# CentaureaHO/CTC-VR

Hardware: AMD Instinct MI355X
Metric: audio-frames/sec, streaming RNN-T greedy decode (higher is better)
Workload: dtype bf16x3; 1 GPU; configs[1]: batch=64/GPU synthetic 10 s 80-dim fbank, streaming chunk=16 (online_rnnt_decode.py semantics), greedy decode, whole-utterance call (tokens identical to the per-chunk API); streams_per_gpu=64, chunk_frames=16, chunks=62, weights=seeded synthetic (seed 0, blank_bias 12.0), parallelism=streams sharded x1, no data-path collective

## Files before the change

### ctc-vr_amd/csrc/api_lifecycle.hip.inc

```

int rnnt_abi_version(void) { return 3; }

const char* rnnt_last_error(const rnnt_ctx* ctx) { return ctx ? ctx->err.c_str() : "null context"; }

int rnnt_create(const rnnt_config* cfg, rnnt_ctx** out) {
    if (!cfg || !out) return RNNT_ERR_ARG;
    *out = nullptr;
    rnnt_ctx* ctx = new rnnt_ctx();
    ctx->cfg = *cfg;
    *out = ctx;
    if (cfg->max_streams < 1 || cfg->max_chunk_frames < 7 || cfg->max_cache_frames < 1 || cfg->max_cache_frames > RNNT_PE_LEN ||
        cfg->max_enc_frames < 1 || cfg->max_tokens < 1 || cfg->vocab_size < 2 || cfg->blank_id < 0 || cfg->blank_id >= cfg->vocab_size ||
        cfg->n_steps < 1 || cfg->max_beam < 0 || cfg->max_beam > 64)
        return fail(ctx, RNNT_ERR_ARG, "rnnt_create: bad config");
    HIPCHK(hipSetDevice(cfg->device));
    if (const char* ng = getenv("RNNT_NO_GRAPH")) ctx->use_graphs = (ng[0] == '1') ? 0 : 1;
    if (const char* pe = getenv("RNNT_PERSISTENT")) ctx->use_persistent = (pe[0] == '0') ? 0 : 1;
    if (const char* me = getenv("RNNT_DEC_MULTI")) ctx->use_multi = (me[0] == '0') ? 0 : 1;
    HIPCHK(hipDeviceGetAttribute(&ctx->n_cus, hipDeviceAttributeMultiprocessorCount, cfg->device));
    if (const char* ae = getenv("RNNT_ATTN_STREAM")) ctx->attn_stream = (ae[0] == '0') ? 0 : 1;
    if (const char* be = getenv("RNNT_BEAM_CHAIN")) ctx->use_beam_chain = (be[0] == '0') ? 0 : 1;
    if (const char* pg = getenv("RNNT_PREFIX_GROUP")) ctx->prefix_group = pg[0] == '1' ? 1 : (pg[0] == '4' ? 4 : 0);
    if (const char* fu = getenv("RNNT_FUSED")) ctx->use_fused = atoi(fu);
    if (const char* fe = getenv("RNNT_FUSE_AFTER_NORM")) ctx->fuse_after_norm = (fe[0] == '0') ? 0 : 1;
// ... 325 lines not shown
        putv(&ctx->whh_il, hh);
        putv(&ctx->wih_il, ih);
        putv(&ctx->b_lstm_il, bb);
        put(&ctx->pred_embed, emb->data.data(), emb->data.size());
        put(&ctx->wpr, wpr->data.data(), wpr->data.size()); put(&ctx->bpr, bpr->data.data(), D);
        put(&ctx->wenc, wen->data.data(), wen->data.size()); put(&ctx->benc, ben->data.data(), D);
        put(&ctx->wpf, wpf->data.data(), wpf->data.size()); put(&ctx->bpf, bpf->data.data(), D);
        put(&ctx->wout, wou->data.data(), wou->data.size()); put(&ctx->bout, bou->data.data(), V);
        std::vector<float> wc((size_t)D * D), bc(D);
        for (int n = 0; n < D; ++n) {
            for (int k = 0; k < D; ++k) {
                double acc = 0.0;
                for (int j = 0; j < D; ++j) acc += (double)wpf->data[(size_t)n * D + j] * (double)wpr->data[(size_t)j * D + k];
                wc[(size_t)n * D + k] = (float)acc;
            }
            double acc = bpf->data[n];
            for (int j = 0; j < D; ++j) acc += (double)wpf->data[(size_t)n * D + j] * (double)bpr->data[j];
            bc[n] = (float)acc;
        }
        putv(&ctx->wjc, wc);
        putv(&ctx->bjc, bc);
        const HostTensor* cw = find(ctx, "ctc_head.ctc_lo.weight");
        const HostTensor* cb = find(ctx, "ctc_head.ctc_lo.bias");
        ctx->wctc = ctx->bctc = nullptr;
        if (cw && cb && cw->dims == std::vector<int64_t>{V, D} && cb->dims == std::vector<int64_t>{V}) {
            put(&ctx->wctc, cw->data.data(), cw->data.size());
            put(&ctx->bctc, cb->data.data(), V);
        }
    }
#undef NEED
    while (blob.size() % 8) blob.push_back(0.f);
    int rc;
    if (ctx->blob.cap != blob.size()) {
        HIPCHK(hipStreamSynchronize(s));
        ctx->blob_hi.release();
        ctx->blob_lo.release();
        if ((rc = reserve_exact(ctx, ctx->blob, blob.size()))) return rc;
    }
    HIPCHK(hipMemcpyAsync(ctx->blob, blob.data(), blob.size() * sizeof(float), hipMemcpyHostToDevice, s));
    for (auto& f : fix) *f.first = ctx->blob + f.second;
    ctx->numerics = RNNT_NUM_F32;
    if (numerics_mode != RNNT_NUMERICS_FP32) {
        if ((rc = reserve(ctx, ctx->blob_hi, blob.size()))) return rc;
        if ((rc = reserve(ctx, ctx->blob_lo, blob.size()))) return rc;
        const long long n8 = (long long)(blob.size() / 8);
        if (numerics_mode == RNNT_NUMERICS_F16X3) hipLaunchKernelGGL(split_planes<true>, dim3(grid_for(n8)), dim3(256), 0, s, ctx->blob, ctx->blob_hi, ctx->blob_lo, n8);
        else hipLaunchKernelGGL(split_planes<false>, dim3(grid_for(n8)), dim3(256), 0, s, ctx->blob, ctx->blob_hi, ctx->blob_lo, n8);
        LAUNCHCHK("split_planes");
    }
    {
        const int nm = numerics_mode;
        const size_t per_w = nm == RNNT_NUMERICS_BF16 ? 8 : 4;
        const size_t layer_w = (size_t)4 * FF * D + 5 * D * D + 2 * D * D;
        const size_t vecs = ((size_t)L * layer_w + (size_t)D * 2304) / per_w;
        if (ctx->fuse_w.cap != vecs) {
            HIPCHK(hipStreamSynchronize(s));
            if ((rc = reserve_exact(ctx, ctx->fuse_w, vecs))) return rc;
        }
        if ((rc = reserve(ctx, ctx->layers_dev, (size_t)L))) return rc;
        std::vector<LayerDev> ld(L);
        uint4* cur = ctx->fuse_w;
        auto pack = [&](const float* W, int N, int K) -> const uint4* {
            const uint4* out = cur;
            const long long total = (long long)((N + 15) / 16) * (K / 32) * 64;
            const dim3 g(grid_for(total)), b(256);
            switch (nm) {
                case RNNT_NUMERICS_BF16X3: hipLaunchKernelGGL(pack_frag<RNNT_NUM_BF16X3>, g, b, 0, s, W, N, K, K, cur); break;
                case RNNT_NUMERICS_BF16: hipLaunchKernelGGL(pack_frag<RNNT_NUM_BF16>, g, b, 0, s, W, N, K, K, cur); break;
                case RNNT_NUMERICS_F16X3: hipLaunchKernelGGL(pack_frag<RNNT_NUM_F16X3>, g, b, 0, s, W, N, K, K, cur); break;
                default: hipLaunchKernelGGL(pack_frag<RNNT_NUM_F32>, g, b, 0, s, W, N, K, K, cur); break;
            }
            cur += (size_t)N * K / per_w;
            return out;
        };
        for (int l = 0; l < L; ++l) {
            const LayerW& w = ctx->lw[l];
            LayerDev& d = ld[l];
            d.w1m = pack(w.w1m, FF, D); d.w2m = pack(w.w2m, D, FF); d.wq = pack(w.wq, D, D); d.wk = pack(w.wk, D, D); d.wv = pack(w.wv, D, D);
            d.wo = pack(w.wo, D, D); d.pw1 = pack(w.pw1, 2 * D, D); d.pw2 = pack(w.pw2, D, D); d.w1 = pack(w.w1, FF, D); d.w2 = pack(w.w2, D, FF);
            d.b1m = w.b1m; d.b2m = w.b2m; d.bq = w.bq; d.bk = w.bk; d.bv = w.bv; d.bo = w.bo; d.bpw1 = w.bpw1; d.bpw2 = w.bpw2; d.b1 = w.b1; d.b2 = w.b2;
            d.ln_ffm_g = w.ln_ffm_g; d.ln_ffm_b = w.ln_ffm_b; d.ln_mha_g = w.ln_mha_g; d.ln_mha_b = w.ln_mha_b; d.ln_conv_g = w.ln_conv_g;
            d.ln_conv_b = w.ln_conv_b; d.ln_ff_g = w.ln_ff_g; d.ln_ff_b = w.ln_ff_b; d.ln_fin_g = w.ln_fin_g; d.ln_fin_b = w.ln_fin_b;
            d.wdw_t = w.wdw_t; d.bdw = w.bdw; d.bn_s = w.bn_s; d.bn_t = w.bn_t;
            d.kc = ctx->kcache + (size_t)l * ctx->cfg.max_streams * ctx->tcap * D;
            d.vc = ctx->vcache + (size_t)l * ctx->cfg.max_streams * ctx->tcap * D;
            d.gr = ctx->gring + (size_t)l * ctx->cfg.max_streams * ctx->cap * D;
            d.xr = ctx->xring + (size_t)l * ctx->cfg.max_streams * ctx->cap * D;
        }
        ctx->conv2_wp = pack(ctx->conv2_w, D, 2304);
        LAUNCHCHK("pack_frag");
        HIPCHK(hipMemcpyAsync(ctx->layers_dev, ld.data(), L * sizeof(LayerDev), hipMemcpyHostToDevice, s));
        ctx->layers_host = ld;
        HIPCHK(hipStreamSynchronize(s));
    }
    if (numerics_mode != RNNT_NUMERICS_FP32 && V <= JR_NT * 16 && V % 4 == 0) {
        const bool lo = numerics_mode != RNNT_NUMERICS_BF16;
        const size_t bytes = (size_t)(lo ? 16 : 8) * JR_SLOT;
        if (ctx->joint_wfrag.cap != bytes) {
            HIPCHK(hipStreamSynchronize(s));
            if ((rc = reserve_exact(ctx, ctx->joint_wfrag, bytes))) return rc;
        }
        if ((rc = reserve(ctx, ctx->joint_counter, (size_t)4))) return rc;
        const dim3 g((unsigned)(bytes / 16 + 255) / 256), b(256);
        if (numerics_mode == RNNT_NUMERICS_F16X3) hipLaunchKernelGGL((pack_joint_w<true, true>), g, b, 0, s, ctx->wout, (int)V, ctx->joint_wfrag);
        else if (lo) hipLaunchKernelGGL((pack_joint_w<false, true>), g, b, 0, s, ctx->wout, (int)V, ctx->joint_wfrag);
        else hipLaunchKernelGGL((pack_joint_w<false, false>), g, b, 0, s, ctx->wout, (int)V, ctx->joint_wfrag);
        LAUNCHCHK("pack_joint_w");
    }
    for (int l = 0; l < L; ++l) {
        if ((rc = reserve(ctx, ctx->ptab[l], (size_t)RNNT_PE_LEN * D))) return rc;
        ctx->lw[l].ptab = ctx->ptab[l];
        GemmP g = plain_gemm(ctx->pe, D, ctx->lw[l].wpos, D, nullptr, ctx->lw[l].ptab, D, RNNT_PE_LEN, D, D);
        if ((rc = launch_gemm(ctx, s, &g, 1))) return rc;
    }
    if ((rc = reserve(ctx, ctx->egate, (size_t)V * 4 * D))) return rc;
    {
        GemmP g = plain_gemm(ctx->pred_embed, D, ctx->wih_il, D, ctx->b_lstm_il, ctx->egate, 4 * D, V, 4 * D, D);
        if ((rc = launch_gemm(ctx, s, &g, 1))) return rc;
    }
    HIPCHK(hipStreamSynchronize(s));
    ctx->numerics = numerics_mode;
    ctx->finalized = true;
    return RNNT_OK;
}

int rnnt_streams_reset(rnnt_ctx* ctx, int32_t n_streams, void* stream) {
    if (!ctx) return RNNT_ERR_ARG;
    if (!ctx->finalized) return fail(ctx, RNNT_ERR_STATE, "weights not finalized");
    if (n_streams < 1 || n_streams > ctx->cfg.max_streams) return fail(ctx, RNNT_ERR_ARG, "n_streams %d out of range", n_streams);
    hipStream_t s = (hipStream_t)stream;
    const int B = ctx->cfg.max_streams;
    ctx->n_streams = n_streams;
    ctx->pos = SlotPos{0, 0, 0};
    ctx->frames_buffered = 0; ctx->frames_decoded = 0;
    ctx->launches = 0; ctx->greedy_steps = 0;
    ctx->pool_mode = false;
    for (PoolSlot& q : ctx->slot) q.pos = SlotPos{0, 0, 0};
    hipLaunchKernelGGL(conv_ring_init, dim3(grid_for((long long)L * B * ctx->cap * D)), dim3(256), 0, s, ctx->gring, ctx->xring, ctx->glu0, B, ctx->cap);
    LAUNCHCHK("conv_ring_init");
    hipLaunchKernelGGL(decode_state_reset, dim3(grid_for((long long)2 * B * D)), dim3(256), 0, s, ctx->h, ctx->c, ctx->sel, ctx->key, ctx->fidx, ctx->nsym,
                       ctx->count, ctx->n_active, ctx->tok, ctx->cfg.blank_id, B);
    LAUNCHCHK("decode_state_reset");
// ... 8 lines not shown
```

### ctc-vr_amd/csrc/host_launch.hip.inc

```

namespace {

int fail(rnnt_ctx* ctx, int code, const char* fmt, ...) {
    char buf[512];
    va_list ap;
    va_start(ap, fmt);
    vsnprintf(buf, sizeof(buf), fmt, ap);
    va_end(ap);
    if (ctx) ctx->err = buf;
    return code;
}

#define HIPCHK(expr)                                                                                   \
    do {                                                                                               \
        hipError_t e_ = (expr);                                                                        \
        if (e_ != hipSuccess) return fail(ctx, RNNT_ERR_HIP, "%s failed: %s", #expr, hipGetErrorString(e_)); \
    } while (0)

#define LAUNCHERR(name)                                                                                \
    do {                                                                                               \
        hipError_t e_ = hipGetLastError();                                                             \
        if (e_ != hipSuccess) return fail(ctx, RNNT_ERR_HIP, "launch %s failed: %s", name, hipGetErrorString(e_)); \
    } while (0)

// ... 310 lines not shown
        const int nq_ = attn_nq(tq);                                                                   \
        const dim3 grid_(gx, ((tq) + 4 * nq_ - 1) / (4 * nq_), gz);                                    \
        if (nq_ == 1) { hipLaunchKernelGGL(KERNEL<1>, grid_, dim3(256), 0, s, __VA_ARGS__); LAUNCHCHK(#KERNEL "<1>"); }      \
        else if (nq_ == 2) { hipLaunchKernelGGL(KERNEL<2>, grid_, dim3(256), 0, s, __VA_ARGS__); LAUNCHCHK(#KERNEL "<2>"); } \
        else { hipLaunchKernelGGL(KERNEL<4>, grid_, dim3(256), 0, s, __VA_ARGS__); LAUNCHCHK(#KERNEL "<4>"); }               \
    } while (0)

int launch_attn(rnnt_ctx* ctx, hipStream_t s, const AttnP& a, int B) {
    ProfScope prof(ctx, s, TAG_ATTN);
    if (attn_stream_ok(ctx, a.tq, a.T2)) {
        const int cap = attn_t2cap(a.T2);
        hipLaunchKernelGGL(rel_attention_stream, dim3(B * RNNT_H), dim3(256), attn_stream_lds(cap), s, a, cap);
        LAUNCHCHK("rel_attention_stream");
        return RNNT_OK;
    }
    LAUNCH_ATTN_TILED(rel_attention, s, B * RNNT_H, a.tq, 1, a);
    return RNNT_OK;
}
int launch_dw(rnnt_ctx* ctx, hipStream_t s, const DwP& d) {
    ProfScope prof(ctx, s, TAG_DWCONV);
    hipLaunchKernelGGL(dwconv_bn_silu, dim3(grid_for((long long)d.B * d.tq * D)), dim3(256), 0, s, d);
    LAUNCHCHK("dwconv_bn_silu");
    return RNNT_OK;
}
int launch_ln(rnnt_ctx* ctx, hipStream_t s, const LnP& p) {
    hipLaunchKernelGGL(layer_norm, dim3((p.M + 3) / 4), dim3(256), 0, s, p);
    LAUNCHCHK("layer_norm");
    return RNNT_OK;
}

int run_layer(rnnt_ctx* ctx, hipStream_t s, int l, int B, int tq, int T2, int kv_row0, int pos_start, int ring_pos,
              const int* klen_dev) {
    LayerDescs d;
    LayerBufs bf{ctx->x, ctx->hbuf, ctx->qbuf, ctx->abuf, ctx->dbuf};
    int rc = build_layer(ctx, l, B, tq, T2, kv_row0, pos_start, ring_pos, klen_dev, bf, d);
    if (rc) return rc;
    if ((rc = launch_gemm(ctx, s, &d.ffn1m, 1, TAG_FFN1))) return rc;
    if ((rc = launch_gemm(ctx, s, &d.ffn2m, 1, TAG_FFN2))) return rc;
    if ((rc = launch_gemm(ctx, s, d.qkv, 3, TAG_QKV))) return rc;
    if ((rc = launch_attn(ctx, s, d.attn, B))) return rc;
    if ((rc = launch_gemm(ctx, s, &d.out, 1, TAG_ATTN_OUT))) return rc;
    if ((rc = launch_gemm(ctx, s, &d.pw1, 1, TAG_PW1))) return rc;
    if ((rc = launch_dw(ctx, s, d.dw))) return rc;
    if ((rc = launch_gemm(ctx, s, &d.pw2, 1, TAG_PW2))) return rc;
    if ((rc = launch_gemm(ctx, s, &d.ffn1, 1, TAG_FFN1))) return rc;
    if ((rc = launch_gemm(ctx, s, &d.ffn2, 1, TAG_FFN2))) return rc;
    return launch_ln(ctx, s, d.lnf);
}

static bool conv2_bw_on(const rnnt_ctx* ctx) { return ctx->conv2_bw != 0; }
static bool conv2_fused(const rnnt_ctx* ctx, long long M) {
    return ctx->conv1_fuse && ctx->numerics != RNNT_NUM_F32 && conv2_bw_on(ctx) && ctx->conv2_wp && M >= 32768 && M < (1ll << 31);
}
int run_subsample(rnnt_ctx* ctx, hipStream_t s, const float* fbank, int B, int Tstride, int T, const int* starts_dev, int nc,
                  float* y1, float* y2, float* xout, int out_cn = 0, int out_rows = 0, int out_r0 = 0, bool minor = false, bool fuse_ok = false) {
    const int tag1 = minor ? TAG_CONV1_MINOR : TAG_CONV1, tag2 = minor ? TAG_CONV2_MINOR : TAG_CONV2, tag3 = minor ? TAG_EMBED_MINOR : TAG_EMBED;
    const int t1 = sub1_len(T), tq = sub_len(T);
    const int VB = nc * B;
    int rc;
    const bool fused = fuse_ok && conv2_fused(ctx, (long long)VB * tq * RNNT_FSUB);
    if (!fused) {
        if (!y1) return fail(ctx, RNNT_ERR_STATE, "run_subsample: no conv1 slab");
        ProfScope prof(ctx, s, tag1);
        if (ctx->conv1_rows && !ctx->gemm_m_cap && (long long)VB * ((t1 + C1_TB - 1) / C1_TB) >= 256) {
            hipLaunchKernelGGL(conv1_relu_rows, dim3(VB, (t1 + C1_TB - 1) / C1_TB), dim3(256), 0, s, fbank, ctx->conv1_wt, ctx->conv1_b, y1, B, Tstride, t1,
                               starts_dev, nc, out_cn > 0 ? 1 : 0);
            LAUNCHCHK("conv1_relu_rows");
        } else {
            hipLaunchKernelGGL(conv1_relu, dim3(grid_for((long long)VB * t1 * RNNT_F1 * D)), dim3(256), 0, s, fbank, ctx->conv1_wt, ctx->conv1_b,
                               y1, B, Tstride, t1, starts_dev, nc, out_cn > 0 ? 1 : 0);
            LAUNCHCHK("conv1_relu");
        }
    }
    GemmP g = plain_gemm(y1, 0, ctx->conv2_w, 2304, ctx->conv2_b, y2, D, VB * tq * RNNT_FSUB, D, 2304, EPI_RELU);
    g.a_n1 = tq * RNNT_FSUB; g.a_n2 = RNNT_FSUB;
    g.a_s0 = (long long)t1 * RNNT_F1 * D; g.a_s1 = 2LL * RNNT_F1 * D; g.a_s2 = 2LL * D;
    g.a_seg = 768; g.a_seg_stride = (long long)RNNT_F1 * D;
    const int conv2_lds = ctx->conv2_lds;
    const bool conv2_bw = conv2_bw_on(ctx);
    const bool nw8 = ctx->bw_nw == 8;
#define BW_LAUNCH_NUM(KERNEL, NUM_, ...) { if (nw8) hipLaunchKernelGGL((KERNEL<NUM_, 8>), grid, dim3(512), 0, s, __VA_ARGS__); \
                                           else hipLaunchKernelGGL((KERNEL<NUM_, 4>), grid, dim3(256), 0, s, __VA_ARGS__); }
#define BW_LAUNCH(KERNEL, ...)                                                                         \
    switch (ctx->numerics) {                                                                           \
        case RNNT_NUM_BF16: BW_LAUNCH_NUM(KERNEL, RNNT_NUM_BF16, __VA_ARGS__) break;                   \
        case RNNT_NUM_F16X3: BW_LAUNCH_NUM(KERNEL, RNNT_NUM_F16X3, __VA_ARGS__) break;                 \
        default: BW_LAUNCH_NUM(KERNEL, RNNT_NUM_BF16X3, __VA_ARGS__) break;                            \
    }                                                                                                  \
    LAUNCHERR(#KERNEL)
    if (fused) {
        ProfScope prof(ctx, s, tag2);
        g.A = nullptr;
        if ((rc = prepare_gemm(ctx, g))) return rc;
        const dim3 grid((g.M + 127) / 128);
        const Conv1Src src{fbank, ctx->conv1_wt, ctx->conv1_b, starts_dev, B, Tstride, nc, out_cn > 0 ? 1 : 0};
        BW_LAUNCH(gemm_bw_c1, g, ctx->conv2_wp, src);
        if (nw8) LAUNCHCHK("gemm_bw_c1<8>"); else LAUNCHCHK("gemm_bw_c1<4>");
    } else if (ctx->numerics != RNNT_NUM_F32 && conv2_bw && ctx->conv2_wp && g.M >= 32768 && !ctx->gemm_m_cap) {
        ProfScope prof(ctx, s, tag2);
        if ((rc = prepare_gemm(ctx, g))) return rc;
        const dim3 grid((g.M + 127) / 128);
        BW_LAUNCH(gemm_bw, g, ctx->conv2_wp);
        if (nw8) LAUNCHCHK("gemm_bw<8>"); else LAUNCHCHK("gemm_bw<4>");
#undef BW_LAUNCH
#undef BW_LAUNCH_NUM
    } else if (ctx->numerics != RNNT_NUM_F32) {
        if ((rc = launch_gemm(ctx, s, &g, 1, tag2))) return rc;
    } else if (conv2_lds && g.M >= 2048 && !ctx->gemm_m_cap) {
        ProfScope prof(ctx, s, tag2);
        GemmBatch gb;
        memset(&gb, 0, sizeof(gb));
        gb.g[0] = g;
        if ((rc = prepare_gemm(ctx, gb.g[0]))) return rc;
        const bool pd1 = prefetch_depth(ctx) == 1;
        if (conv2_lds == 2 && nc > 1) { launch_gemm_ns<2, 2, false, true>(ctx, s, gb, g.M, g.N, 1); if (pd1) LAUNCHCHK("gemm_ns<2,2,nt;pd1>"); else LAUNCHCHK("gemm_ns<2,2,nt>"); }
        else { launch_gemm_ns<2, 2>(ctx, s, gb, g.M, g.N, 1); if (pd1) LAUNCHCHK("gemm_ns<2,2;pd1>"); else LAUNCHCHK("gemm_ns<2,2>"); }
    } else if ((rc = launch_gemm(ctx, s, &g, 1, tag2))) return rc;
    GemmP go = plain_gemm(y2, RNNT_FSUB * D, ctx->emb_w, RNNT_FSUB * D, ctx->emb_b, xout, D, VB * tq, D, RNNT_FSUB * D, EPI_SCALE, 16.0f);
    if (out_cn > 0) { go.c_n = out_cn; go.c_s0 = (long long)out_rows * D; go.c_r0 = out_r0; go.c_mod = BIG; go.c_s1 = D; }
    return launch_gemm(ctx, s, &go, 1, tag3);
}

template <int NUM>
size_t fuse_lds(int MT, bool back) {
    const size_t R = 16 * MT, opb = FuseCfg<NUM>::OPB;
    return back ? R * 1024 + R * opb + R * 1024 + sizeof(FuseRows) : R * 1024 + 2 * R * opb + sizeof(FuseRows);
}
template <int NUM, int MT>
int launch_fused_t(rnnt_ctx* ctx, hipStream_t s, bool back, const FuseItem* tab, int n_items, int n_groups, int S, int B) {
    const size_t lds = fuse_lds<NUM>(MT, back);
    int rc_attr;
    const dim3 grid((unsigned)((n_items + 7) / 8 * 8 * n_groups));
    if (back) {
        if ((rc_attr = ensure_dyn_lds(ctx, reinterpret_cast<const void*>(&block_back<NUM, MT>), lds))) return rc_attr;
        hipLaunchKernelGGL((block_back<NUM, MT>), grid, dim3(FUSE_THREADS), lds, s, ctx->layers_dev, tab, ctx->wf_x, n_items, n_groups, S, B, ctx->cap);
        if (MT == 1) LAUNCHCHK("block_back<1>"); else if (MT == 2) LAUNCHCHK("block_back<2>"); else LAUNCHCHK("block_back<3>");
    } else {
        if ((rc_attr = ensure_dyn_lds(ctx, reinterpret_cast<const void*>(&block_front<NUM, MT>), lds))) return rc_attr;
        hipLaunchKernelGGL((block_front<NUM, MT>), grid, dim3(FUSE_THREADS), lds, s, ctx->layers_dev, tab, ctx->wf_x, n_items, n_groups, S, B, (long long)ctx->tcap);
        if (MT == 1) LAUNCHCHK("block_front<1>"); else if (MT == 2) LAUNCHCHK("block_front<2>"); else LAUNCHCHK("block_front<3>");
    }
    return RNNT_OK;
}
template <int NUM>
int launch_fused_n(rnnt_ctx* ctx, hipStream_t s, bool back, const FuseItem* tab, int n_items, int n_groups, int S, int B, int MT) {
    switch (MT) {
        case 1: return launch_fused_t<NUM, 1>(ctx, s, back, tab, n_items, n_groups, S, B);
        case 2: return launch_fused_t<NUM, 2>(ctx, s, back, tab, n_items, n_groups, S, B);
        default: return launch_fused_t<NUM, 3>(ctx, s, back, tab, n_items, n_groups, S, B);
    }
}
int launch_fused(rnnt_ctx* ctx, hipStream_t s, bool back, const FuseItem* tab, int n_items, int maxnf, int B, int tag) {
    ProfScope prof(ctx, s, tag);
    int S = FUSE_ROWS / maxnf;
    if (S > B) S = B;
    if (S < 1) return fail(ctx, RNNT_ERR_SHAPE, "fused block: %d frames per stream exceed the %d-row tile", maxnf, FUSE_ROWS);
    const int n_groups = (B + S - 1) / S, MT = (S * maxnf + 15) / 16;
    switch (ctx->numerics) {
        case RNNT_NUM_BF16X3: return launch_fused_n<RNNT_NUM_BF16X3>(ctx, s, back, tab, n_items, n_groups, S, B, MT);
        case RNNT_NUM_BF16: return launch_fused_n<RNNT_NUM_BF16>(ctx, s, back, tab, n_items, n_groups, S, B, MT);
        case RNNT_NUM_F16X3: return launch_fused_n<RNNT_NUM_F16X3>(ctx, s, back, tab, n_items, n_groups, S, B, MT);
        default: return launch_fused_n<RNNT_NUM_F32>(ctx, s, back, tab, n_items, n_groups, S, B, MT);
    }
}

template <int WK, int MT, int NT>
void launch_gemm16_tab(hipStream_t s, const GemmP* tab, int n, int maxM, int maxN) {
    dim3 grid((maxN + 16 * NT - 1) / (16 * NT), (maxM + 16 * MT - 1) / (16 * MT), n);
    hipLaunchKernelGGL((gemm16_tab<WK, MT, NT>), grid, dim3(64 * WK), 0, s, tab);
}
int launch_gemm_tab(rnnt_ctx* ctx, hipStream_t s, const GemmP* tab_dev, int n, int maxM, int N, int K, int tag) {
    ProfScope prof(ctx, s, tag);
// ... 296 lines not shown
```

### ctc-vr_amd/csrc/host_lm.hip.inc

```

namespace {

struct LmPlan { bool ok; int c_r0, c_mod, park0; };
LmPlan lm_plan(const rnnt_ctx* ctx, const std::vector<ChunkInfo>& ci, int F) {
    LmPlan p{false, 0, BIG, -1};
    const int C = (int)ci.size();
    auto wrow = [&](int c) { return ci[c].kv_w0(); };
    bool contiguous = true;
    for (int c = 1; c < C; ++c) contiguous = contiguous && wrow(c) == wrow(c - 1) + ci[c - 1].tq;
    if (contiguous) { p.ok = true; p.c_r0 = wrow(0); return p; }
    bool tail_contig = C >= 2 && wrow(1) == 0 && ci[0].T2 == ci[0].tq && wrow(0) == 0;
    for (int c = 2; c < C; ++c) tail_contig = tail_contig && wrow(c) == wrow(c - 1) + ci[c - 1].tq;
    if (tail_contig && F <= ctx->tcap) {
        p.ok = true; p.c_r0 = ctx->tcap - ci[0].tq; p.c_mod = ctx->tcap; p.park0 = ctx->tcap - ci[0].tq;
        return p;
    }
    return p;
}

struct RaggedPlan {
    std::vector<int> nb;
    std::vector<ChunkInfo> tail;
    std::vector<int> frames;
    int F = 0;
};

int lm_res_upload(rnnt_ctx* ctx, hipStream_t s, const std::vector<std::vector<LmRow>>& tabs) {
    ctx->lm_res_ok = 0;
    if (!lm_res_plan(tabs, ctx->lm_rhdr_host, ctx->lm_rrows_host, ctx->lm_res_stride)) return RNNT_OK;
    int rc;
    if ((rc = reserve(ctx, ctx->lm_rhdr, ctx->lm_rhdr_host.size()))) return rc;
    if ((rc = reserve(ctx, ctx->lm_rrows, ctx->lm_rrows_host.size()))) return rc;
    HIPCHK(hipMemcpyAsync(ctx->lm_rhdr, ctx->lm_rhdr_host.data(), ctx->lm_rhdr_host.size() * sizeof(LmResHdr), hipMemcpyHostToDevice, s));
    HIPCHK(hipMemcpyAsync(ctx->lm_rrows, ctx->lm_rrows_host.data(), ctx->lm_rrows_host.size() * sizeof(LmRow), hipMemcpyHostToDevice, s));
    ctx->lm_res_ok = 1;
    return RNNT_OK;
}

constexpr int AS_MT = 3;
template <int NUM>
int launch_gemm_as_t(rnnt_ctx* ctx, hipStream_t s, const AsBatch& ab) {
    const size_t lds = (size_t)FuseCfg<NUM>::PLANES * 16 * AS_MT * FuseCfg<NUM>::ROWB;
    { const int rc_attr = ensure_dyn_lds(ctx, reinterpret_cast<const void*>(&gemm_as<NUM, AS_MT>), lds); if (rc_attr) return rc_attr; }
    hipLaunchKernelGGL((gemm_as<NUM, AS_MT>), dim3((ab.g[0].M + 16 * AS_MT - 1) / (16 * AS_MT)), dim3(256), lds, s, ab);
    LAUNCHCHK("gemm_as");
    return RNNT_OK;
}
int launch_gemm_as(rnnt_ctx* ctx, hipStream_t s, const GemmP* gs, const uint4* const* wp, int ng, int tag) {
    ProfScope prof(ctx, s, tag);
    AsBatch ab;
    memset(&ab, 0, sizeof(ab));
    ab.ng = ng;
    for (int i = 0; i < ng; ++i) {
        ab.g[i] = gs[i];
        ab.wp[i] = wp[i];
        int rc = prepare_gemm(ctx, ab.g[i]);
        if (rc) return rc;
        if (gs[i].N % 64 || gs[i].M != gs[0].M || gs[i].K != gs[0].K || gs[i].A != gs[0].A) return fail(ctx, RNNT_ERR_SHAPE, "gemm_as: descriptors do not share A / shape");
    }
    const int K = gs[0].K;
    if (!(K == 256 || (K % 256 == 0 && ng == 1 && gs[0].N == 256)) || !ab.g[0].a_plain) return fail(ctx, RNNT_ERR_SHAPE, "gemm_as: unsupported shape K=%d N=%d", K, gs[0].N);
    switch (ctx->numerics) {
        case RNNT_NUM_BF16X3: return launch_gemm_as_t<RNNT_NUM_BF16X3>(ctx, s, ab);
        case RNNT_NUM_F16X3: return launch_gemm_as_t<RNNT_NUM_F16X3>(ctx, s, ab);
        case RNNT_NUM_BF16: return launch_gemm_as_t<RNNT_NUM_BF16>(ctx, s, ab);
        default: return fail(ctx, RNNT_ERR_STATE, "gemm_as: exact-f32 mode has no packed 16-bit weights");
    }
}
template <int NUM, int NW>
int launch_ffn_as_t(rnnt_ctx* ctx, hipStream_t s, const FfnP& p) {
    const size_t lds = FFN_LDS(NUM, NW) + ((p.H0 || p.dw.g || p.w1p2) ? FFN_XROWS : 0);
    { const int rc_attr = ensure_dyn_lds(ctx, reinterpret_cast<const void*>(&ffn_as<NUM, AS_MT, NW>), lds); if (rc_attr) return rc_attr; }
    hipLaunchKernelGGL((ffn_as<NUM, AS_MT, NW>), dim3((p.M + 16 * AS_MT - 1) / (16 * AS_MT)), dim3(64 * NW), lds, s, p);
    if (NW == 16) LAUNCHCHK("ffn_as<16>"); else if (NW == 4) LAUNCHCHK("ffn_as<4>"); else LAUNCHCHK("ffn_as<8>");
    return RNNT_OK;
}
int launch_ffn_as(rnnt_ctx* ctx, hipStream_t s, const FfnP& p) {
    ProfScope prof(ctx, s, p.A0 ? TAG_OUT_PW1 : (p.w1p2 ? TAG_FFN_MERGED : (p.n_tail > 0 ? TAG_FFN_QKV : TAG_FFN_FUSED)));
    const int nw = ctx->ffn_nw;
#define FFN_NW_DISPATCH(NUM_) return nw == 16 ? launch_ffn_as_t<NUM_, 16>(ctx, s, p) : nw == 4 ? launch_ffn_as_t<NUM_, 4>(ctx, s, p) : launch_ffn_as_t<NUM_, 8>(ctx, s, p)
    switch (ctx->numerics) {
        case RNNT_NUM_BF16X3: FFN_NW_DISPATCH(RNNT_NUM_BF16X3);
        case RNNT_NUM_F16X3: FFN_NW_DISPATCH(RNNT_NUM_F16X3);
        case RNNT_NUM_BF16: FFN_NW_DISPATCH(RNNT_NUM_BF16);
        default: return fail(ctx, RNNT_ERR_STATE, "ffn_as: exact-f32 mode has no packed 16-bit weights");
    }
}

int encoder_chunks_lm(rnnt_ctx* ctx, hipStream_t s, const float* fbank_dev, int total_frames, const int32_t* chunk_start,
                      const std::vector<ChunkInfo>& ci, const std::vector<int>& plan_key, int greedy, bool* handled,
                      float* out_plain = nullptr, const int* klen_dev = nullptr, const RaggedPlan* rg = nullptr) {
    *handled = false;
    if (!ctx->use_lm) return RNNT_OK;
    const int B = ctx->n_streams, C = (int)ci.size(), Bm = ctx->cfg.max_streams;
    const int fb0 = ci[0].fpos;
    int F = 0;
    for (int c = 0; c < C; ++c) F += ci[c].tq;
    if (rg) F = std::max(F, rg->F);
    const LmPlan plan = lm_plan(ctx, ci, F);
    if (!plan.ok) return RNNT_OK;
    const long long M = (long long)B * F;
    if (M * RNNT_FSUB >= (1ll << 31)) return RNNT_OK;
    int rc;
    const int fmax = std::max(ctx->fcap, ctx->tmax);
    if (F > fmax) return RNNT_OK;
    const int gs = RNNT_LORDER + fmax;
    const size_t rows = (size_t)Bm * fmax;
    if ((rc = reserve(ctx, ctx->lm_x, rows * D))) return rc;
    if ((rc = reserve(ctx, ctx->lm_h, rows * FF))) return rc;
    if ((rc = reserve(ctx, ctx->lm_q, rows * D))) return rc;
    if ((rc = reserve(ctx, ctx->lm_a, rows * D))) return rc;
    if ((rc = reserve(ctx, ctx->lm_d, rows * D))) return rc;
    if ((rc = reserve(ctx, ctx->lm_g, (size_t)L * Bm * gs * D))) return rc;
    float* x = ctx->lm_x;
    bool ctx_in_done = false;
    struct SideJoin {
        rnnt_ctx* ctx; hipStream_t s; bool armed;
        ~SideJoin() {
// ... 368 lines not shown
```

### ctc-vr_amd/csrc/rnnt_api.hip

```cpp
#include "rnnt_kernels.hip.h"
#include "../../include/rnnt_hip.h"

#include <climits>
#include <cmath>
#include <cstdarg>
#include <cstdio>
#include <chrono>
#include <cstdlib>
#include <cstring>
#include <functional>
#include <map>
#include <string>
#include <unordered_map>
#include <algorithm>
#include <array>
#include <atomic>
#include <vector>

namespace {

constexpr int D = RNNT_D, FF = RNNT_FF, L = RNNT_L, DK = RNNT_DK;
constexpr int BIG = INT_MAX;

struct LayerW {
// ... 63 lines not shown
    size_t cap = 0;
    DevBuf() = default;
    DevBuf(const DevBuf&) = delete;
    DevBuf& operator=(const DevBuf&) = delete;
    ~DevBuf() { release(); }
    void release() {
        if (p && HOST) (void)hipHostFree(p);
        else if (p) { (void)hipFree(p); live_device_bytes -= (int64_t)(cap * sizeof(T)); }
        p = nullptr;
        cap = 0;
    }
    operator T*() const { return p; }
};
template <typename T>
using PinnedBuf = DevBuf<T, true>;

struct SearchSlot { int frames_done, beam; float cw, tw; int use_context; int64_t gen; int use_ngram; int64_t ngen; };
struct WvSlot { int samples, frames, rate, nfft, finished; };
struct HsSlot { int keep, len; };
struct SegSlot { int index, start, frames; };
struct PoolSlot {
    SlotPos pos{0, 0, 0};
    int beam_cur = 0, beam_lbound = 0, prefix_cur = 0;
    SearchSlot ctc{}, prefix{};
    WvSlot wave{};
    HsSlot hist{};
    int ep = 0;
    SegSlot seg{};
};
struct CallTab {
    DevBuf<int> dev;
    PinnedBuf<int> host;
    hipEvent_t ev = nullptr;
    ~CallTab() { if (ev) (void)hipEventDestroy(ev); }
    operator int*() const { return dev.p; }
};

enum WfType { WF_FFN1M, WF_FFN2M, WF_QKV, WF_OUT, WF_PW1, WF_PW2, WF_FFN1, WF_FFN2, WF_ATTN, WF_DW, WF_LN, WF_BLOCK_FRONT, WF_BLOCK_BACK };

}

struct rnnt_ctx {
    rnnt_config cfg;
    std::string err;
    std::map<std::string, HostTensor> host;
    bool finalized = false;
    int numerics = 0;

    DevBuf<float> blob;
    DevBuf<unsigned short> blob_hi, blob_lo;
    DevBuf<uint4> fuse_w;
    DevBuf<LayerDev> layers_dev;
    const uint4* conv2_wp = nullptr;
    DevBuf<unsigned char> joint_wfrag;
    DevBuf<int> joint_counter;
    std::map<const void*, int> dyn_lds;
    std::vector<LayerDev> layers_host;
    int use_as = 1;
    int use_fused = 1;
    DevBuf<FuseItem> wf_ftab;
    int wf_fused_plan = 0;
    LayerW lw[L];
    DevBuf<float> ptab[L];
    const float *conv1_wt, *conv1_b, *conv2_w, *conv2_b, *emb_w, *emb_b, *pe, *after_g, *after_b;
    const float *ln_conv_g_all, *ln_conv_b_all, *glu0;
    const float *whh_il, *wih_il, *b_lstm_il, *pred_embed, *wpr, *bpr, *wenc, *benc, *wpf, *bpf, *wout, *bout;
    DevBuf<float> egate;

    int tmax = 0, t1max = 0, cap = 0, tcap = 0, fcap = 0, fstride = 0, vpad = 0;
    DevBuf<float> y1, y2, x, hbuf, qbuf, abuf, dbuf;
    DevBuf<float> kcache, vcache, gring, xring;
    DevBuf<float> encbuf, encp;
    DevBuf<float> h, c, pred, z, logits;
    DevBuf<int> tok, fidx, nsym, count, tokens, n_active, klen, sel;
    DevBuf<unsigned long long> key;
    DevBuf<int> dec_ctrl;
    int use_persistent = 1;
    int attn_stream = 1;
    int fuse_after_norm = 1;
    int overlap_ok = -1;
    int use_multi = 1;
    int n_cus = 0;
    DevBuf<unsigned long long> gm_x1, gm_xa;
    DevBuf<long long> gm_dbg;
    int gm_dbg_rows = 0;
    const float *wjc = nullptr, *bjc = nullptr;
    const float *wctc = nullptr, *bctc = nullptr;
    int max_rows = 0;
    DevBuf<float> pool[2], bpred, bz, blogits, b_blank, b_toplp;
    DevBuf<int> b_tok, b_frame, b_active, b_steps, b_toptok, b_srcrow, b_srcstep;
    int pool_cur = 0;
    PinnedBuf<int> pinned;
    DevBuf<float> scratch;

    int n_streams = 0;
    SlotPos pos{0, 0, 0};
    int frames_buffered = 0, frames_decoded = 0;
    int64_t launches = 0, greedy_steps = 0;
    std::vector<PoolSlot> slot;
    bool pool_mode = false;
    CallTab pool_tab;
    int gemm_m_cap = 0;
    DevBuf<float> wf_x, wf_h, wf_q, wf_a, wf_d, wf_y1, wf_y2;
    int wf_slab = 0;
    DevBuf<int> wf_starts;
    DevBuf<GemmP> wf_gtab; DevBuf<AttnP> wf_atab; DevBuf<DwP> wf_dtab; DevBuf<LnP> wf_ltab;
// ... 144 lines not shown
```

### ctc-vr_amd/csrc/rnnt_gemm_as.hip.h

```cpp
#pragma once

#ifdef AS_TRACE
__device__ long long as_trace[4096 * 8];
#define AS_STAMP(k_) { if (lane == 0 && blockIdx.x < 1024) as_trace[(blockIdx.x * 4 + wave) * 8 + (k_)] = (long long)__builtin_amdgcn_s_memrealtime(); }
#else
#define AS_STAMP(k_)
#endif
#define AS_MT_ 3
#ifndef BW_WD
#define BW_WD 3
#endif
#ifndef BW_ABL
#define BW_ABL 0
#endif
#ifndef FFN_ABL2
#define FFN_ABL2 0
#endif
struct AsBatch {
    GemmP g[3];
    const uint4* wp[3];
    int ng;
};

template <int MT, int NTW = 4>
__device__ __forceinline__ void as_epilogue_t(const GemmP& p, const f32x4_ (&acc)[MT][NTW], int m0, int n0, int lane) {
    const int i = lane & 15, q = lane >> 4;
    const int epi = p.epi;
    float4 bias[NTW];
#pragma unroll
    for (int t = 0; t < NTW; ++t) bias[t] = p.bias ? ldg4(p.bias + n0 + 16 * t + 4 * q) : make_float4(0.f, 0.f, 0.f, 0.f);
#pragma unroll
    for (int mt = 0; mt < MT; ++mt) {
        const int m = m0 + 16 * mt + i;
        if (m >= p.M) continue;
        const long long crow = c_row_off(p, m);
#pragma unroll
        for (int t = 0; t < NTW; ++t) {
            const int n = n0 + 16 * t + 4 * q;
            float4 v = make_float4(acc[mt][t][0] + bias[t].x, acc[mt][t][1] + bias[t].y, acc[mt][t][2] + bias[t].z, acc[mt][t][3] + bias[t].w);
            if (epi == EPI_GLU) {
                *reinterpret_cast<float2*>(p.C + crow + (n >> 1)) = make_float2(v.x * sigmoidf_(v.y), v.z * sigmoidf_(v.w));
                continue;
            }
            if (epi == EPI_SILU) { v.x *= sigmoidf_(v.x); v.y *= sigmoidf_(v.y); v.z *= sigmoidf_(v.z); v.w *= sigmoidf_(v.w); }
            else if (epi == EPI_RELU) { v.x = fmaxf(v.x, 0.f); v.y = fmaxf(v.y, 0.f); v.z = fmaxf(v.z, 0.f); v.w = fmaxf(v.w, 0.f); }
            else if (epi == EPI_SCALE) { v.x *= p.alpha; v.y *= p.alpha; v.z *= p.alpha; v.w *= p.alpha; }
            else if (epi == EPI_RESID) {
                const float4 r4 = ldg4(p.R + crow + n);
                v.x = r4.x + p.alpha * v.x; v.y = r4.y + p.alpha * v.y; v.z = r4.z + p.alpha * v.z; v.w = r4.w + p.alpha * v.w;
            }
            stg4(p.C + crow + n, v);
        }
    }
}

template <int NUM, int MT>
__global__ __launch_bounds__(256) void gemm_as(AsBatch P) {
    using C = FuseCfg<NUM>;
    constexpr bool F16 = C::F16, LO = C::PLANES == 2;
    constexpr int U = C::PLANES, R = 16 * MT, ROWB = C::ROWB;
    extern __shared__ __attribute__((aligned(16))) unsigned char as_op[];
    const int tid = threadIdx.x, lane = tid & 63, wave = tid >> 6;
    const int i = lane & 15, q = lane >> 4;
    const int bm0 = blockIdx.x * R;
    const GemmP& p0 = P.g[0];
    if (bm0 >= p0.M) return;
    const int KP = p0.K >> 8;
    const unsigned char* rowp[MT];
#pragma unroll
    for (int mt = 0; mt < MT; ++mt) rowp[mt] = as_op + (16 * mt + i) * ROWB;

    auto stage = [&](int kp) {
        if (p0.ln_g) {
            constexpr int NP = R / 16;
            const int g = lane >> 4, l16 = lane & 15;
            float4 v[NP][4];
#pragma unroll
            for (int ps = 0; ps < NP; ++ps) {
                const float* rp = p0.A + a_row_off(p0, min(bm0 + wave * 4 + g + 16 * ps, p0.M - 1));
#pragma unroll
                for (int j = 0; j < 2; ++j) { v[ps][2 * j] = ldg4(rp + 8 * (l16 + 16 * j)); v[ps][2 * j + 1] = ldg4(rp + 8 * (l16 + 16 * j) + 4); }
            }
            float mu[NP], rs[NP];
#pragma unroll
            for (int ps = 0; ps < NP; ++ps) {
                float sm = 0.f;
#pragma unroll
                for (int j = 0; j < 4; ++j) sm += (v[ps][j].x + v[ps][j].y) + (v[ps][j].z + v[ps][j].w);
#pragma unroll
                for (int o = 8; o > 0; o >>= 1) sm += __shfl_xor(sm, o, 16);
                mu[ps] = sm * (1.0f / 256.0f);
            }
#pragma unroll
            for (int ps = 0; ps < NP; ++ps) {
                float qq = 0.f;
#pragma unroll
                for (int j = 0; j < 4; ++j) {
                    const float dx = v[ps][j].x - mu[ps], dy = v[ps][j].y - mu[ps], dz = v[ps][j].z - mu[ps], dw = v[ps][j].w - mu[ps];
                    qq += (dx * dx + dy * dy) + (dz * dz + dw * dw);
                }
#pragma unroll
                for (int o = 8; o > 0; o >>= 1) qq += __shfl_xor(qq, o, 16);
                rs[ps] = 1.0f / sqrtf(qq * (1.0f / 256.0f) + 1e-5f);
            }
#pragma unroll
            for (int j = 0; j < 2; ++j) {
                const int c = l16 + 16 * j;
                const float4 g0 = ldg4(p0.ln_g + 8 * c), g1 = ldg4(p0.ln_g + 8 * c + 4), b0_ = ldg4(p0.ln_b + 8 * c), b1_ = ldg4(p0.ln_b + 8 * c + 4);
#pragma unroll
                for (int ps = 0; ps < NP; ++ps) {
                    const int r = wave * 4 + g + 16 * ps;
                    const float m_ = mu[ps], s_ = rs[ps];
                    float4 x0 = v[ps][2 * j], x1 = v[ps][2 * j + 1];
                    x0.x = (x0.x - m_) * s_ * g0.x + b0_.x; x0.y = (x0.y - m_) * s_ * g0.y + b0_.y; x0.z = (x0.z - m_) * s_ * g0.z + b0_.z; x0.w = (x0.w - m_) * s_ * g0.w + b0_.w;
                    x1.x = (x1.x - m_) * s_ * g1.x + b1_.x; x1.y = (x1.y - m_) * s_ * g1.y + b1_.y; x1.z = (x1.z - m_) * s_ * g1.z + b1_.z; x1.w = (x1.w - m_) * s_ * g1.w + b1_.w;
                    uint4 h, l;
                    split8_16<F16, LO>(x0, x1, h, l);
                    const int off = op_off<NUM>(r, c);
                    *reinterpret_cast<uint4*>(as_op + off) = h;
                    if constexpr (LO) *reinterpret_cast<uint4*>(as_op + R * ROWB + off) = l;
                }
            }
        } else {
            constexpr int CJ = R * 32 / 256;
            float4 va[CJ], vb[CJ];
#pragma unroll
            for (int j = 0; j < CJ; ++j) {
                const int e = tid + 256 * j, r = e >> 5, c = e & 31;
                const float* ap = p0.A + a_row_off(p0, min(bm0 + r, p0.M - 1)) + (kp << 8) + 8 * c;
                va[j] = ldg4(ap);
                vb[j] = ldg4(ap + 4);
            }
#pragma unroll
            for (int j = 0; j < CJ; ++j) {
                const int e = tid + 256 * j, r = e >> 5, c = e & 31;
                uint4 h, l;
                split8_16<F16, LO>(va[j], vb[j], h, l);
                const int off = op_off<NUM>(r, c);
                *reinterpret_cast<uint4*>(as_op + off) = h;
                if constexpr (LO) *reinterpret_cast<uint4*>(as_op + R * ROWB + off) = l;
            }
        }
    };
    auto bload = [&](uint4 (&b)[4 * U], const uint4* __restrict__ Wp, int KT, int grp, int kt) {
#pragma unroll
        for (int t = 0; t < 4; ++t)
#pragma unroll
            for (int u = 0; u < U; ++u) {
#if defined(__HIP_DEVICE_COMPILE__)
                typedef unsigned u32x4g_ __attribute__((ext_vector_type(4)));
                const u32x4g_ v = *(const RNNT_GAS u32x4g_*)(Wp + ((long long)((grp * 4 + t) * KT + kt) * U + u) * 64 + lane);
                b[t * U + u] = make_uint4(v[0], v[1], v[2], v[3]);
#else
                b[t * U + u] = Wp[((long long)((grp * 4 + t) * KT + kt) * U + u) * 64 + lane];
#endif
            }
    };
    auto mma = [&](f32x4_ (&acc)[MT][4], const uint4 (&b)[4 * U], int ks) {
        uint4 ah[MT], al[LO ? MT : 1];
#pragma unroll
        for (int mt = 0; mt < MT; ++mt) {
            const int off = ((4 * ks + q) ^ i) << 4;
            ah[mt] = *reinterpret_cast<const uint4*>(rowp[mt] + off);
            if constexpr (LO) al[mt] = *reinterpret_cast<const uint4*>(rowp[mt] + R * ROWB + off);
        }
#pragma unroll
        for (int t = 0; t < 4; ++t)
#pragma unroll
            for (int mt = 0; mt < MT; ++mt) {
                if constexpr (LO) {
                    acc[mt][t] = mfma16_<F16>(b[t * U], al[mt], acc[mt][t]);
                    acc[mt][t] = mfma16_<F16>(b[t * U + 1], ah[mt], acc[mt][t]);
                }
                acc[mt][t] = mfma16_<F16>(b[t * U], ah[mt], acc[mt][t]);
            }
        __builtin_amdgcn_sched_barrier(0);
    };
    f32x4_ acc[MT][4];
    uint4 b0[4 * U], b1[4 * U];
    auto zero = [&]() {
#pragma unroll
        for (int mt = 0; mt < MT; ++mt)
#pragma unroll
            for (int t = 0; t < 4; ++t) acc[mt][t] = (f32x4_){0.f, 0.f, 0.f, 0.f};
    };

    if (KP > 1) {
        const int KT = p0.K >> 5;
        const uint4* Wp = P.wp[0];
        zero();
        bload(b0, Wp, KT, wave, 0);
        for (int kp = 0; kp < KP; ++kp) {
            if (kp) __syncthreads();
            stage(kp);
            __syncthreads();
#pragma unroll
            for (int ks = 0; ks < 8; ks += 2) {
                const int kt = kp * 8 + ks;
                bload(b1, Wp, KT, wave, kt + 1);
                mma(acc, b0, ks);
                if (kt + 2 < KT) bload(b0, Wp, KT, wave, kt + 2);
                mma(acc, b1, ks + 1);
            }
        }
        as_epilogue_t<MT>(p0, acc, bm0, wave * 64, lane);
        return;
    }
    AS_STAMP(0)
    stage(0);
    AS_STAMP(1)
    __syncthreads();
    AS_STAMP(2)
    int gi = 0, grp = wave;
    while (gi < P.ng && grp * 64 >= P.g[gi].N) { ++gi; grp = wave; }
    if (gi < P.ng) bload(b0, P.wp[gi], 8, grp, 0);
    while (gi < P.ng) {
        int ngi = gi, ngrp = grp + 4;
        while (ngi < P.ng && ngrp * 64 >= P.g[ngi].N) { ++ngi; ngrp = wave; }
        zero();
        const uint4* Wp = P.wp[gi];
#pragma unroll
        for (int ks = 0; ks < 8; ks += 2) {
            bload(b1, Wp, 8, grp, ks + 1);
            mma(acc, b0, ks);
            if (ks + 2 < 8) bload(b0, Wp, 8, grp, ks + 2);
            else if (ngi < P.ng) bload(b0, P.wp[ngi], 8, ngrp, 0);
            mma(acc, b1, ks + 1);
        }
        AS_STAMP(3)
        as_epilogue_t<MT>(P.g[gi], acc, bm0, grp * 64, lane);
        AS_STAMP(4)
        gi = ngi; grp = ngrp;
    }
}

struct FfnP {
    const float* X;
    float* Y;
    const float *ln_g, *ln_b;
    const uint4 *w1p, *w2p;
    const float *b1, *b2;
    const float *lno_g, *lno_b;
    float alpha;
    int M;
    const float *ln_g2, *ln_b2;
    const uint4 *w1p2, *w2p2;
    const float *b1_2, *b2_2;
    float alpha2;
    int n_tail;
    const float *lnt_g, *lnt_b;
    const float* A0;
    const float* H0;
    DwLmP dw;
    const uint4* whp;
    const float* bh;
    const int* hrowlen;
    int hrowlen_n;
    GemmP tg[3];
    const uint4* twp[3];
};
#define FFN_TIMG 51200
#define FFN_FLD 260
#ifndef FFN_KU
#define FFN_KU 2
#endif

#define FFN_LDS(NUM_, NW_) ((size_t)FFN_TIMG + (size_t)FuseCfg<NUM_>::PLANES * 16 * AS_MT_ * FuseCfg<NUM_>::ROWB)
#define FFN_XROWS (16 * AS_MT_ * FFN_FLD * 4)
template <int NUM, int MT, int NW = 4>
__global__ __launch_bounds__(64 * NW) void ffn_as(FfnP P) {
    constexpr int NTW = 16 / NW, CW = 16 * NTW, NT = 64 * NW;
    using C = FuseCfg<NUM>;
    constexpr bool F16 = C::F16, LO = C::PLANES == 2;
    constexpr int U = C::PLANES, R = 16 * MT, ROWB = C::ROWB, IMG = U * R * ROWB;
    extern __shared__ __attribute__((aligned(16))) unsigned char ffn_smem[];
    unsigned char* Xop = ffn_smem;
    unsigned char* Hop = ffn_smem + IMG;
    const int tid = threadIdx.x, lane = tid & 63, wave = tid >> 6;
    const int i = lane & 15, q = lane >> 4;
    const int bm0 = blockIdx.x * R;
    if (bm0 >= P.M) return;
    float* fin = reinterpret_cast<float*>(ffn_smem);
    static_assert(R * FFN_FLD * 4 <= FFN_TIMG && 2 * IMG <= FFN_TIMG + IMG, "result rows / both images must fit FFN_LDS");
    auto bload = [&](uint4 (&b)[NTW * U], const uint4* __restrict__ Wp, int KT, int ct0 , int kt) {
#if FFN_ABL2 & 1
        for (int t = 0; t < NTW * U; ++t) b[t] = make_uint4(0x3c003c00u + lane, 0x3c003c00u, 0x3c003c00u, 0x3c003c00u);
// ... 642 lines not shown
```

Measured before the change: 14.52 million audio-frames/s.

## Route embed GEMM through packed-weight AS kernel with double-buffered K-panel pipeline

```diff
diff --git a/ctc-vr_amd/csrc/api_lifecycle.hip.inc b/ctc-vr_amd/csrc/api_lifecycle.hip.inc
--- a/ctc-vr_amd/csrc/api_lifecycle.hip.inc
+++ b/ctc-vr_amd/csrc/api_lifecycle.hip.inc
@@ -401,7 +401,7 @@
         const int nm = numerics_mode;
         const size_t per_w = nm == RNNT_NUMERICS_BF16 ? 8 : 4;
         const size_t layer_w = (size_t)4 * FF * D + 5 * D * D + 2 * D * D;
-        const size_t vecs = ((size_t)L * layer_w + (size_t)D * 2304) / per_w;
+        const size_t vecs = ((size_t)L * layer_w + (size_t)D * 2304 + (size_t)D * RNNT_FSUB * D) / per_w;
         if (ctx->fuse_w.cap != vecs) {
             HIPCHK(hipStreamSynchronize(s));
             if ((rc = reserve_exact(ctx, ctx->fuse_w, vecs))) return rc;
@@ -437,6 +437,7 @@
             d.xr = ctx->xring + (size_t)l * ctx->cfg.max_streams * ctx->cap * D;
         }
         ctx->conv2_wp = pack(ctx->conv2_w, D, 2304);
+        ctx->emb_wp = pack(ctx->emb_w, D, RNNT_FSUB * D);
         LAUNCHCHK("pack_frag");
         HIPCHK(hipMemcpyAsync(ctx->layers_dev, ld.data(), L * sizeof(LayerDev), hipMemcpyHostToDevice, s));
         ctx->layers_host = ld;
diff --git a/ctc-vr_amd/csrc/host_launch.hip.inc b/ctc-vr_amd/csrc/host_launch.hip.inc
--- a/ctc-vr_amd/csrc/host_launch.hip.inc
+++ b/ctc-vr_amd/csrc/host_launch.hip.inc
@@ -386,6 +386,11 @@
 static bool conv2_fused(const rnnt_ctx* ctx, long long M) {
     return ctx->conv1_fuse && ctx->numerics != RNNT_NUM_F32 && conv2_bw_on(ctx) && ctx->conv2_wp && M >= 32768 && M < (1ll << 31);
 }
+constexpr int EMBED_AS_MIN_ROWS = 4096;
+static bool embed_as(const rnnt_ctx* ctx, int M) {
+    return ctx->numerics != RNNT_NUM_F32 && ctx->use_as && ctx->emb_wp && !ctx->gemm_m_cap && M >= EMBED_AS_MIN_ROWS;
+}
+int launch_gemm_as(rnnt_ctx* ctx, hipStream_t s, const GemmP* gs, const uint4* const* wp, int ng, int tag);
 int run_subsample(rnnt_ctx* ctx, hipStream_t s, const float* fbank, int B, int Tstride, int T, const int* starts_dev, int nc,
                   float* y1, float* y2, float* xout, int out_cn = 0, int out_rows = 0, int out_r0 = 0, bool minor = false, bool fuse_ok = false) {
     const int tag1 = minor ? TAG_CONV1_MINOR : TAG_CONV1, tag2 = minor ? TAG_CONV2_MINOR : TAG_CONV2, tag3 = minor ? TAG_EMBED_MINOR : TAG_EMBED;
@@ -452,6 +457,7 @@
     } else if ((rc = launch_gemm(ctx, s, &g, 1, tag2))) return rc;
     GemmP go = plain_gemm(y2, RNNT_FSUB * D, ctx->emb_w, RNNT_FSUB * D, ctx->emb_b, xout, D, VB * tq, D, RNNT_FSUB * D, EPI_SCALE, 16.0f);
     if (out_cn > 0) { go.c_n = out_cn; go.c_s0 = (long long)out_rows * D; go.c_r0 = out_r0; go.c_mod = BIG; go.c_s1 = D; }
+    if (embed_as(ctx, go.M)) return launch_gemm_as(ctx, s, &go, &ctx->emb_wp, 1, tag3);
     return launch_gemm(ctx, s, &go, 1, tag3);
 }
 
diff --git a/ctc-vr_amd/csrc/host_lm.hip.inc b/ctc-vr_amd/csrc/host_lm.hip.inc
--- a/ctc-vr_amd/csrc/host_lm.hip.inc
+++ b/ctc-vr_amd/csrc/host_lm.hip.inc
@@ -46,6 +46,15 @@
     LAUNCHCHK("gemm_as");
     return RNNT_OK;
 }
+constexpr int AS_KP_NW = 8;
+template <int NUM>
+int launch_gemm_as_kp_t(rnnt_ctx* ctx, hipStream_t s, const AsBatch& ab) {
+    const size_t lds = (size_t)2 * FuseCfg<NUM>::PLANES * 16 * AS_MT * FuseCfg<NUM>::ROWB;
+    { const int rc_attr = ensure_dyn_lds(ctx, reinterpret_cast<const void*>(&gemm_as_kp<NUM, AS_MT, AS_KP_NW>), lds); if (rc_attr) return rc_attr; }
+    hipLaunchKernelGGL((gemm_as_kp<NUM, AS_MT, AS_KP_NW>), dim3((ab.g[0].M + 16 * AS_MT - 1) / (16 * AS_MT)), dim3(64 * AS_KP_NW), lds, s, ab.g[0], ab.wp[0]);
+    LAUNCHCHK("gemm_as");
+    return RNNT_OK;
+}
 int launch_gemm_as(rnnt_ctx* ctx, hipStream_t s, const GemmP* gs, const uint4* const* wp, int ng, int tag) {
     ProfScope prof(ctx, s, tag);
     AsBatch ab;
@@ -60,10 +69,11 @@
     }
     const int K = gs[0].K;
     if (!(K == 256 || (K % 256 == 0 && ng == 1 && gs[0].N == 256)) || !ab.g[0].a_plain) return fail(ctx, RNNT_ERR_SHAPE, "gemm_as: unsupported shape K=%d N=%d", K, gs[0].N);
+    const bool kp = K > 256;
     switch (ctx->numerics) {
-        case RNNT_NUM_BF16X3: return launch_gemm_as_t<RNNT_NUM_BF16X3>(ctx, s, ab);
-        case RNNT_NUM_F16X3: return launch_gemm_as_t<RNNT_NUM_F16X3>(ctx, s, ab);
-        case RNNT_NUM_BF16: return launch_gemm_as_t<RNNT_NUM_BF16>(ctx, s, ab);
+        case RNNT_NUM_BF16X3: return kp ? launch_gemm_as_kp_t<RNNT_NUM_BF16X3>(ctx, s, ab) : launch_gemm_as_t<RNNT_NUM_BF16X3>(ctx, s, ab);
+        case RNNT_NUM_F16X3: return kp ? launch_gemm_as_kp_t<RNNT_NUM_F16X3>(ctx, s, ab) : launch_gemm_as_t<RNNT_NUM_F16X3>(ctx, s, ab);
+        case RNNT_NUM_BF16: return kp ? launch_gemm_as_kp_t<RNNT_NUM_BF16>(ctx, s, ab) : launch_gemm_as_t<RNNT_NUM_BF16>(ctx, s, ab);
         default: return fail(ctx, RNNT_ERR_STATE, "gemm_as: exact-f32 mode has no packed 16-bit weights");
     }
 }
diff --git a/ctc-vr_amd/csrc/rnnt_api.hip b/ctc-vr_amd/csrc/rnnt_api.hip
--- a/ctc-vr_amd/csrc/rnnt_api.hip
+++ b/ctc-vr_amd/csrc/rnnt_api.hip
@@ -139,6 +139,7 @@
     DevBuf<uint4> fuse_w;
     DevBuf<LayerDev> layers_dev;
     const uint4* conv2_wp = nullptr;
+    const uint4* emb_wp = nullptr;
     DevBuf<unsigned char> joint_wfrag;
     DevBuf<int> joint_counter;
     std::map<const void*, int> dyn_lds;
diff --git a/ctc-vr_amd/csrc/rnnt_gemm_as.hip.h b/ctc-vr_amd/csrc/rnnt_gemm_as.hip.h
--- a/ctc-vr_amd/csrc/rnnt_gemm_as.hip.h
+++ b/ctc-vr_amd/csrc/rnnt_gemm_as.hip.h
@@ -65,12 +65,11 @@
     const int bm0 = blockIdx.x * R;
     const GemmP& p0 = P.g[0];
     if (bm0 >= p0.M) return;
-    const int KP = p0.K >> 8;
     const unsigned char* rowp[MT];
 #pragma unroll
     for (int mt = 0; mt < MT; ++mt) rowp[mt] = as_op + (16 * mt + i) * ROWB;
 
-    auto stage = [&](int kp) {
+    auto stage = [&]() {
         if (p0.ln_g) {
             constexpr int NP = R / 16;
             const int g = lane >> 4, l16 = lane & 15;
@@ -127,7 +126,7 @@
 #pragma unroll
             for (int j = 0; j < CJ; ++j) {
                 const int e = tid + 256 * j, r = e >> 5, c = e & 31;
-                const float* ap = p0.A + a_row_off(p0, min(bm0 + r, p0.M - 1)) + (kp << 8) + 8 * c;
+                const float* ap = p0.A + a_row_off(p0, min(bm0 + r, p0.M - 1)) + 8 * c;
                 va[j] = ldg4(ap);
                 vb[j] = ldg4(ap + 4);
             }
@@ -185,29 +184,8 @@
             for (int t = 0; t < 4; ++t) acc[mt][t] = (f32x4_){0.f, 0.f, 0.f, 0.f};
     };
 
-    if (KP > 1) {
-        const int KT = p0.K >> 5;
-        const uint4* Wp = P.wp[0];
-        zero();
-        bload(b0, Wp, KT, wave, 0);
-        for (int kp = 0; kp < KP; ++kp) {
-            if (kp) __syncthreads();
-            stage(kp);
-            __syncthreads();
-#pragma unroll
-            for (int ks = 0; ks < 8; ks += 2) {
-                const int kt = kp * 8 + ks;
-                bload(b1, Wp, KT, wave, kt + 1);
-                mma(acc, b0, ks);
-                if (kt + 2 < KT) bload(b0, Wp, KT, wave, kt + 2);
-                mma(acc, b1, ks + 1);
-            }
-        }
-        as_epilogue_t<MT>(p0, acc, bm0, wave * 64, lane);
-        return;
-    }
     AS_STAMP(0)
-    stage(0);
+    stage();
     AS_STAMP(1)
     __syncthreads();
     AS_STAMP(2)
@@ -232,6 +210,102 @@
         AS_STAMP(4)
         gi = ngi; grp = ngrp;
     }
+}
+
+#define AS_WD 3
+template <int NUM, int MT, int NW>
+__global__ __launch_bounds__(64 * NW) void gemm_as_kp(GemmP p, const uint4* __restrict__ Wp) {
+    using C = FuseCfg<NUM>;
+    constexpr bool F16 = C::F16, LO = C::PLANES == 2;
+    constexpr int U = C::PLANES, R = 16 * MT, ROWB = C::ROWB, IMG = U * R * ROWB, NTW = 16 / NW, NT = 64 * NW;
+    constexpr int CJ = R * 32 / NT;
+    constexpr int CD = 8 - CJ;
+    static_assert(R * 32 % NT == 0 && CJ >= 1 && CJ <= 6, "row chunks per thread: loads in k-steps 0 .. CJ - 1, stores from k-step CD >= 2 on");
+    extern __shared__ __attribute__((aligned(16))) unsigned char kp_op[];
+    const int tid = threadIdx.x, lane = tid & 63, wave = tid >> 6;
+    const int i = lane & 15, q = lane >> 4;
+    const int bm0 = blockIdx.x * R;
+    if (bm0 >= p.M) return;
+    const int KP = p.K >> 8, KT = p.K >> 5;
+    const float* ap[CJ];
+    int aoff[CJ];
+#pragma unroll
+    for (int j = 0; j < CJ; ++j) {
+        const int e = tid + NT * j, r = e >> 5, c = e & 31;
+        ap[j] = p.A + a_row_off(p, min(bm0 + r, p.M - 1)) + 8 * c;
+        aoff[j] = op_off<NUM>(r, c);
+    }
+    float4 va[CJ], vb[CJ];
+    auto aload = [&](int j, int kp) { va[j] = ldg4_nt(ap[j] + (kp << 8)); vb[j] = ldg4_nt(ap[j] + (kp << 8) + 4); };
+    auto astore = [&](int j, unsigned char* op) {
+        uint4 h, l;
+        split8_16<F16, LO>(va[j], vb[j], h, l);
+        *reinterpret_cast<uint4*>(op + aoff[j]) = h;
+        if constexpr (LO) *reinterpret_cast<uint4*>(op + R * ROWB + aoff[j]) = l;
+    };
+    auto bload = [&](uint4 (&b)[NTW * U], int kt) {
+#pragma unroll
+        for (int t = 0; t < NTW; ++t)
+#pragma unroll
+            for (int u = 0; u < U; ++u) {
+#if defined(__HIP_DEVICE_COMPILE__)
+                typedef unsigned u32x4g_ __attribute__((ext_vector_type(4)));
+                const u32x4g_ v = *(const RNNT_GAS u32x4g_*)(Wp + ((long long)((wave * NTW + t) * KT + kt) * U + u) * 64 + lane);
+                b[t * U + u] = make_uint4(v[0], v[1], v[2], v[3]);
+#else
+                b[t * U + u] = Wp[((long long)((wave * NTW + t) * KT + kt) * U + u) * 64 + lane];
+#endif
+            }
+    };
+    f32x4_ acc[MT][NTW];
+#pragma unroll
+    for (int mt = 0; mt < MT; ++mt)
+#pragma unroll
+        for (int t = 0; t < NTW; ++t) acc[mt][t] = (f32x4_){0.f, 0.f, 0.f, 0.f};
+    auto mma = [&](const uint4 (&b)[NTW * U], int ks, const unsigned char* op) {
+        uint4 ah[MT], al[LO ? MT : 1];
+#pragma unroll
+        for (int mt = 0; mt < MT; ++mt) {
+            const unsigned char* rp = op + (16 * mt + i) * ROWB + (((4 * ks + q) ^ i) << 4);
+            ah[mt] = *reinterpret_cast<const uint4*>(rp);
+            if constexpr (LO) al[mt] = *reinterpret_cast<const uint4*>(rp + R * ROWB);
+        }
+#pragma unroll
+        for (int t = 0; t < NTW; ++t)
+#pragma unroll
+            for (int mt = 0; mt < MT; ++mt) {
+                if constexpr (LO) {
+                    acc[mt][t] = mfma16_<F16>(b[t * U], al[mt], acc[mt][t]);
+                    acc[mt][t] = mfma16_<F16>(b[t * U + 1], ah[mt], acc[mt][t]);
+                }
+                acc[mt][t] = mfma16_<F16>(b[t * U], ah[mt], acc[mt][t]);
+            }
+        __builtin_amdgcn_sched_barrier(0);
+    };
+    uint4 wb[4][NTW * U];
+#pragma unroll
+    for (int k = 0; k < AS_WD; ++k) bload(wb[k], k);
+#pragma unroll
+    for (int j = 0; j < CJ; ++j) aload(j, 0);
+#pragma unroll
+    for (int j = 0; j < CJ; ++j) astore(j, kp_op);
+    __syncthreads();
+#pragma unroll 1
+    for (int kp = 0; kp < KP; ++kp) {
+        const unsigned char* cur = kp_op + (kp & 1) * IMG;
+        unsigned char* nxt = kp_op + ((kp + 1) & 1) * IMG;
+        const int kpn = min(kp + 1, KP - 1);
+#pragma unroll
+        for (int ks = 0; ks < 8; ++ks) {
+            const int kt = kp * 8 + ks;
+            bload(wb[(ks + AS_WD) & 3], min(kt + AS_WD, KT - 1));
+            if (ks < CJ) aload(ks, kpn);
+            mma(wb[ks & 3], ks, cur);
+            if (ks >= CD) astore(ks - CD, nxt);
+        }
+        __syncthreads();
+    }
+    as_epilogue_t<MT, NTW>(p, acc, bm0, wave * 16 * NTW, lane);
 }
 
 struct FfnP {
```

Result: faster. 14.69 million audio-frames/s, median of 6 (+1.1%).
